# Lumina-Group/libzkp

Hardware: AMD Instinct MI355X
Metric: proofs/sec (whole node) + ms/proof p50, 4096-proof mixed batch (range / equality / membership / improvement) per MI355X (higher is better)
Workload: dtype u32/u64 integer limbs (10x25.5-bit GF(2^255-19), BN254 Fq on 9x29-bit limbs in the MSM loops and 10x26-bit elsewhere, 8x32-bit Fr and scalars mod l, 2x64-bit f128)

## Files before the change

### libzkp_amd/csrc/bn254_g.h

```cpp
#pragma once
#include "bn254_fq.h"
#include "bn254_fq9.h"

namespace zkp {

struct fq2 { fq c0, c1; };

ZKP_HD inline fq f_add(const fq& a, const fq& b) { return fq_add(a, b); }
ZKP_HD inline fq f_sub(const fq& a, const fq& b) { return fq_sub(a, b); }
ZKP_HD inline fq f_mul(const fq& a, const fq& b) { return fq_mul(a, b); }
ZKP_HD inline fq f_sq(const fq& a) { return fq_sq(a); }
ZKP_HD inline fq f_neg(const fq& a) { return fq_neg(a); }
ZKP_HD inline fq f_dbl(const fq& a) { return fq_dbl(a); }
ZKP_HD inline bool f_is_zero(const fq& a) { return fq_is_zero(a); }
ZKP_HD inline fq f_select(bool c, const fq& a, const fq& b) { return fq_select(c, a, b); }
ZKP_HD inline void f_set_zero(fq& a) { a = fq_zero(); }
ZKP_HD inline void f_set_one(fq& a) { a = fq_one(); }
ZKP_HD inline fq f_inv(const fq& a) { return fq_inv(a); }

ZKP_HD inline fq2 f_add(const fq2& a, const fq2& b) { return fq2{fq_add(a.c0, b.c0), fq_add(a.c1, b.c1)}; }
ZKP_HD inline fq2 f_sub(const fq2& a, const fq2& b) { return fq2{fq_sub(a.c0, b.c0), fq_sub(a.c1, b.c1)}; }
ZKP_HD inline fq2 f_neg(const fq2& a) { return fq2{fq_neg(a.c0), fq_neg(a.c1)}; }
ZKP_HD inline fq2 f_dbl(const fq2& a) { return fq2{fq_dbl(a.c0), fq_dbl(a.c1)}; }
ZKP_HD inline fq2 f_mul(const fq2& a, const fq2& b) {
// ... 224 lines not shown
    return h;
}
ZKP_HD inline void fr_glv_split(const uint32_t k[8], glv_half& h1, glv_half& h2) {
    const uint32_t G1[3] = {0xc7e0b3d7u, 0xd91d232eu, 0x00000002u}, G2[5] = {0x391eb18du, 0x7a7bd9d4u, 0xa773d2cfu, 0x4ccef014u, 0x00000002u};
    const uint32_t A1[2] = {0x94d213e3u, 0x89d32568u}, A2[4] = {0x1221250bu, 0x0be4e154u, 0xeeb859fdu, 0x6f4d8248u};
    const uint32_t NB1[4] = {0x7d4f1128u, 0x8211bbebu, 0xeeb859fcu, 0x6f4d8248u}, B2[2] = {0x94d213e3u, 0x89d32568u};
    uint32_t t1[11], t2[13];
    mp_mul_lo<8, 3, 11>(t1, k, G1); mp_mul_lo<8, 5, 13>(t2, k, G2);
    const uint32_t* c1 = t1 + 8;
    const uint32_t* c2 = t2 + 8;
    uint32_t p11[5], p22[5], p12[5], p21[5];
    mp_mul_lo<3, 2, 5>(p11, c1, A1); mp_mul_lo<5, 4, 5>(p22, c2, A2); mp_mul_lo<3, 4, 5>(p12, c1, NB1); mp_mul_lo<5, 2, 5>(p21, c2, B2);
    uint32_t k1[5], k2[5]; int64_t b1 = 0, b2 = 0;
    ZKP_UNROLL for (int i = 0; i < 5; i++) {
        b1 += (int64_t)k[i] - (int64_t)p11[i] - (int64_t)p22[i]; k1[i] = (uint32_t)b1; b1 >>= 32;
        b2 += (int64_t)p12[i] - (int64_t)p21[i]; k2[i] = (uint32_t)b2; b2 >>= 32;
    }
    h1 = glv_from_160(k1); h2 = glv_from_160(k2);
}
ZKP_HD inline fq fq_glv_beta() {
    const uint32_t w[8] = {0x77fffffeu, 0x57634731u, 0xacdb5c4fu, 0xd4f263f1u, 0xa0d48bacu, 0x59e26bceu, 0x00000000u, 0x00000000u};
    return fq_from_raw(w);
}
template <class F> ZKP_HD inline Jac<F> jac_mul_u128_signed(const Jac<F>& p, const uint32_t mag[4], bool neg) {
    Jac<F> tbl[8];
    tbl[0] = p; tbl[1] = jac_dbl(p);
    for (int i = 2; i < 8; i++) tbl[i] = jac_add(tbl[i - 1], p);
    int dig[33]; int carry = 0;
    for (int i = 0; i < 32; i++) {
        int v = (int)((mag[i >> 3] >> ((i & 7) * 4)) & 15u) + carry;
        carry = v > 8 ? 1 : 0; if (carry) v -= 16;
        dig[i] = v;
    }
    dig[32] = carry;
    Jac<F> acc = jac_infinity<F>();
    for (int i = 32; i >= 0; i--) {
        if (i != 32) acc = jac_dbl(jac_dbl(jac_dbl(jac_dbl(acc))));
        const int d = dig[i];
        if (d > 0) acc = jac_add(acc, tbl[d - 1]);
        else if (d < 0) acc = jac_add(acc, jac_neg(tbl[-d - 1]));
    }
    return neg ? jac_neg(acc) : acc;
}

template <class F> ZKP_HD inline bool jac_to_aff(Aff<F>& out, const Jac<F>& p) {
    if (jac_is_inf(p)) return false;
    const F zi = f_inv(p.Z), zi2 = f_sq(zi);
    out.x = f_mul(p.X, zi2); out.y = f_mul(f_mul(p.Y, zi2), zi);
    return true;
}

ZKP_HD inline bool fq_raw_gt_half(const uint32_t w[8]) {
    const uint32_t half[8] = {0x6c3e7ea3u, 0x9e10460bu, 0xb438e546u, 0xcbc0b548u, 0x40c0ac2eu, 0xdc2822dbu, 0x7098d014u, 0x18322739u};
    for (int i = 7; i >= 0; i--) { if (w[i] > half[i]) return true; if (w[i] < half[i]) return false; }
    return false;
}
ZKP_HD inline void g1_serialize(uint32_t out[16], const g1_jac& p) {
    g1_aff a;
    if (!jac_to_aff(a, p)) { for (int i = 0; i < 16; i++) out[i] = 0; out[15] = 0x40000000u; return; }
    fq_to_raw(out, a.x); fq_to_raw(out + 8, a.y);
    if (fq_raw_gt_half(out + 8)) out[15] |= 0x80000000u;
}
ZKP_HD inline void g2_serialize(uint32_t out[32], const g2_jac& p) {
    g2_aff a;
    if (!jac_to_aff(a, p)) { for (int i = 0; i < 32; i++) out[i] = 0; out[31] = 0x40000000u; return; }
// ... 8 lines not shown
```

### libzkp_amd/csrc/g16_impl.inc

```

namespace {

struct G16Key {
    bool loaded = false;
    uint32_t n_inst = 0, n_wit = 0, nv = 0, n_rows = 0, m = 0, logm = 0;
    G16Circuit C{};
    std::vector<void*> allocs;
    uint32_t *table_g1 = nullptr, *table_g2 = nullptr;
    G16Radix rx = g16_radix(G16_WBITS_DEFAULT);
    int shared_tables = -1;
    uint64_t table_bytes = 0;
    struct Chunking { DevLayout lay; const uint32_t* corr = nullptr; const uint16_t* scal = nullptr; };
    std::vector<SlotList> targets_g1, targets_g2;
    std::vector<uint16_t> hscal_g1, hscal_g2;
    std::map<uint64_t, Chunking> lays_g1, lays_g2;
    uint64_t win_g1 = 0, win_g2 = 0;
    const uint32_t *init_g1 = nullptr, *init_g2 = nullptr;
    G16Vk vk{}; bool vk_ready = false;
    uint64_t vk_table_bytes = 0;
    bool verifier_only() const { return vk_ready && !loaded; }
    const uint32_t *vm_kconst = nullptr, *vm_lines = nullptr;
};
struct G16Run {
    void* buf = nullptr; size_t cap = 0; hipStream_t side = nullptr, side2 = nullptr; hipEvent_t ev[4] = {nullptr, nullptr, nullptr, nullptr};
// ... 453 lines not shown
    hipEvent_t e1 = nullptr;
    int rc = prof_begin(K, st, &e1);
    if (rc) return rc;
    ZKP_TRACED(g2 ? "k_msm_gather<G2Msm>" : "k_msm_gather<G1Msm>", st, g16_launch_msm(g2, m, st));
    prof_end(K, st, e1, D.adds_per_row * rows);
    return 0;
}


int run_g16(int kind, uint32_t rows, const uint64_t* d_value, const uint64_t* d_set_vals, const uint32_t* d_set_len, const uint8_t* d_seeds,
            uint8_t* d_out, uint64_t stride, hipStream_t st, uint32_t lane = 0) {
    G16Key& K = g16s().key[kind];
    if (!K.loaded) return no_proving_key(K);
    const uint32_t nsc = g16_nscalars(K.nv, K.m);
    const G16Key::Chunking *c1 = nullptr, *c1c = nullptr, *c2 = nullptr;
    int rc;
    if ((rc = get_chunking(K, false, G16_PART_AB, rows, &c1)) || (rc = get_chunking(K, true, G16_PART_ALL, rows, &c2))) return rc;
    if ((rc = get_chunking(K, false, G16_PART_C, rows, &c1c))) return rc;
    size_t off = 0;
    auto sz = [&](size_t bytes) { size_t o = off; off += align_up(bytes); return o; };
    const size_t W = (size_t)32 * rows;
    const size_t o_z = sz(W * K.nv), o_sd = sz((size_t)K.rx.digw * 4 * rows * nsc), o_rs = sz(W * 2), o_p1 = sz((size_t)c1->lay.nchunks * G1_JAC_W * 4 * rows),
                 o_p1c = sz((size_t)c1c->lay.nchunks * G1_JAC_W * 4 * rows), o_p2 = sz((size_t)c2->lay.nchunks * G2_JAC_W * 4 * rows),
                 o_s1 = sz((size_t)3 * G1_JAC_W * 4 * rows), o_s2 = sz((size_t)G2_JAC_W * 4 * rows), o_t1 = sz((size_t)G16_CPARTS * G1_JAC_W * 4 * rows),
                 o_qe = sz((size_t)2 * 9 * K.m * 4 * rows);
    G16Run& RW = g16s().run[kind][lane & 1u];
    if (off > RW.cap) {
        if (RW.buf) { HIP_TRY(hipDeviceSynchronize()); HIP_TRY(hipFree(RW.buf)); RW.buf = nullptr; RW.cap = 0; }
        HIP_TRY(hipMalloc(&RW.buf, off)); RW.cap = off;
    }
    uint8_t* base = (uint8_t*)RW.buf;
    G16View V{}; V.rx = K.rx; V.rows = rows; V.kind = (uint32_t)kind; V.n_inst = K.n_inst; V.n_wit = K.n_wit; V.nv = K.nv; V.m = K.m;
    V.value = d_value; V.set_vals = d_set_vals; V.set_len = d_set_len; V.seeds = reinterpret_cast<const uint32_t*>(d_seeds); V.mimc_c = g16s().mimc_dev;
    V.z = (uint32_t*)(base + o_z); V.sdig = (uint32_t*)(base + o_sd); V.rs = (uint32_t*)(base + o_rs); V.out = d_out; V.stride = stride;
    V.qap_evals = (uint32_t*)(base + o_qe);
    uint32_t *p1 = (uint32_t*)(base + o_p1), *p1c = (uint32_t*)(base + o_p1c), *p2 = (uint32_t*)(base + o_p2), *s1 = (uint32_t*)(base + o_s1), *s2 = (uint32_t*)(base + o_s2), *t1 = (uint32_t*)(base + o_t1);
    if (!RW.last) {
        for (auto& e : RW.ev) HIP_TRY(hipEventCreateWithFlags(&e, hipEventDisableTiming));
        HIP_TRY(hipEventCreateWithFlags(&RW.last, hipEventDisableTiming));
    }
    G16Run& R0 = g16s().run[kind][0];
    if (!R0.side) {
        static const int side_level = env_int("ZKP_HIP_G16_SIDE_PRIORITY", 2), side2_level = env_int("ZKP_HIP_G16_SIDE2_PRIORITY", 0);
        HIP_TRY(hipStreamCreateWithPriority(&R0.side, hipStreamNonBlocking, stream_priority(side_level)));
        HIP_TRY(hipStreamCreateWithPriority(&R0.side2, hipStreamNonBlocking, stream_priority(side2_level)));
    }
    hipStream_t const side = R0.side, side2 = R0.side2;
    hipEvent_t ev_wit = RW.ev[0], ev_ab = RW.ev[1], ev_c = RW.ev[2], ev_cp = RW.ev[3];
    ReduceView R2{}; R2.rows = rows; R2.ntargets = 1; R2.partial = p2; R2.target_chunk_begin = c2->lay.target_chunk_begin; R2.corr = c2->corr;
    if (RW.used) HIP_TRY(hipStreamWaitEvent(st, RW.last, 0));
    ZKP_TRACED("k_g16_witness", st, g16_launch_witness(V, st));
    ZKP_TRACED("k_g16_zdigits", st, g16_launch_zdigits(V, st));
    HIP_TRY(hipEventRecord(ev_wit, st));
    HIP_TRY(hipStreamWaitEvent(side, ev_wit, 0));
    { TraceMark tm_("k_g16_qap", side); HIP_TRY(g16_launch_qap(V, K.C, side)); }
    if ((rc = launch_msm_key(false, K.rx, *c1c, K.table_g1, K.init_g1, rows, V.sdig, p1c, side))) return rc;
    ReduceView Rc{}; Rc.rows = rows; Rc.ntargets = 1; Rc.partial = p1c; Rc.target_chunk_begin = c1c->lay.target_chunk_begin; Rc.corr = c1c->corr;
    ZKP_TRACED("k_sum_t<G1Msm>", side, g16_launch_sum(false, Rc, s1 + (size_t)2 * G1_JAC_W * rows, side));
    HIP_TRY(hipEventRecord(ev_c, side));
    if ((rc = launch_msm_key(false, K.rx, *c1, K.table_g1, K.init_g1, rows, V.sdig, p1, st))) return rc;
    ReduceView Rab{}; Rab.rows = rows; Rab.ntargets = 2; Rab.partial = p1; Rab.target_chunk_begin = c1->lay.target_chunk_begin; Rab.corr = c1->corr;
    HIP_TRY(hipEventRecord(ev_ab, st));
    HIP_TRY(hipStreamWaitEvent(side2, ev_ab, 0));
    ZKP_TRACED("k_sum_t<G1Msm>", side2, g16_launch_sum(false, Rab, s1, side2));
    ZKP_TRACED("k_g16_cparts", side2, g16_launch_cparts(V, s1, t1, side2));
    HIP_TRY(hipEventRecord(ev_cp, side2));
    if ((rc = launch_msm_key(true, K.rx, *c2, K.table_g2, K.init_g2, rows, V.sdig, p2, st))) return rc;
    ZKP_TRACED("k_sum_t<G2Msm>", st, g16_launch_sum(true, R2, s2, st));
    HIP_TRY(hipStreamWaitEvent(st, ev_c, 0));
    HIP_TRY(hipStreamWaitEvent(st, ev_cp, 0));
    ZKP_TRACED("k_g16_final", st, g16_launch_final(V, s1, s2, t1, st));
    HIP_TRY(hipGetLastError());
    HIP_TRY(hipEventRecord(RW.last, st)); RW.used = true;
    return 0;
}
// ... 243 lines not shown
```

### libzkp_amd/csrc/g16_kernels.hip

```cpp
#include "g16_launch.h"
#include "msm_kernel.h"

struct G1Msm {
    static constexpr uint32_t ACC_W = G1_JAC_W, DIG_PER_WORD = 2;
    static __device__ __forceinline__ int32_t digit(uint32_t word, uint32_t w) { return (int32_t)(int16_t)(word >> (16 * (w & 1u))); }
    using Acc = g1_jac;
    static __device__ __forceinline__ Acc identity() { return jac_infinity<fq>(); }
    static constexpr uint32_t GATHER_WAVES = 3; static constexpr int GATHER_PREFETCH = 2;
    static constexpr uint32_t GATHER_W = 16, GATHER_STRIDE = 16, GATHER_PRIO = 0;
    using GAcc = g1_xyzz9;
    static __device__ __forceinline__ GAcc to_gather(const g1_jac& a) { return xyzz9_from_jac(a); }
    static __device__ __forceinline__ g1_jac from_gather(const GAcc& a) { return jac_from_xyzz9(a); }
    static __device__ __forceinline__ GAcc accumulate_entry(const GAcc& acc, int32_t d, const uint32_t* e) {
        g1_aff9 q{fq9_unpack8(e), fq9_unpack8(e + 8)};
        q.y = fq9_select(d < 0, fq9_neg_k<4>(q.y), q.y);
        return g1_mmadd9(acc, q);
    }
    static __device__ __forceinline__ void store(uint32_t* p, uint32_t idx, uint32_t row, uint32_t rows, const Acc& a) { st_g1_jac(p, idx, row, rows, a); }
    static __device__ __forceinline__ Acc load(const uint32_t* p, uint32_t idx, uint32_t row, uint32_t rows) { return ld_g1_jac(p, idx, row, rows); }
    static __device__ __forceinline__ Acc add(const Acc& a, const Acc& b) { return jac_add(a, b); }
};
struct G2Msm {
    static constexpr uint32_t ACC_W = G2_JAC_W, DIG_PER_WORD = 2;
    static __device__ __forceinline__ int32_t digit(uint32_t word, uint32_t w) { return (int32_t)(int16_t)(word >> (16 * (w & 1u))); }
    using Acc = g2_jac;
    static __device__ __forceinline__ Acc identity() { return jac_infinity<fq2>(); }
    static constexpr uint32_t GATHER_WAVES = 2; static constexpr int GATHER_PREFETCH = -1;
    static constexpr uint32_t GATHER_W = 32, GATHER_STRIDE = 32, GATHER_PRIO = 0;
    using GAcc = g2_xyzz9;
    static __device__ __forceinline__ GAcc to_gather(const g2_jac& a) { return g2_xyzz9_from_jac(a); }
    static __device__ __forceinline__ g2_jac from_gather(const GAcc& a) { return jac_from_g2_xyzz9(a); }
    static __device__ __forceinline__ GAcc accumulate_entry(const GAcc& acc, int32_t d, const uint32_t* e) {
        const g2_aff9 q{fq2_9{fq9_unpack8(e), fq9_unpack8(e + 8)}, fq2_9{fq9_unpack8(e + 16), fq9_unpack8(e + 24)}};
        return g2_mmadd9(acc, q, d < 0);
    }
    static __device__ __forceinline__ void store(uint32_t* p, uint32_t idx, uint32_t row, uint32_t rows, const Acc& a) { st_g2_jac(p, idx, row, rows, a); }
    static __device__ __forceinline__ Acc load(const uint32_t* p, uint32_t idx, uint32_t row, uint32_t rows) { return ld_g2_jac(p, idx, row, rows); }
    static __device__ __forceinline__ Acc add(const Acc& a, const Acc& b) { return jac_add(a, b); }
};


__global__ void __launch_bounds__(TW) k_g16_witness(G16View V) {
    ZKP_RAISE_PRIO();
    const uint32_t row = blockIdx.x * TW + threadIdx.x;
    if (row < V.rows) step_g16_witness(V, row);
}
__global__ void __launch_bounds__(TB) k_g16_zdigits(G16View V) {
    ZKP_RAISE_PRIO();
    const uint32_t row = blockIdx.x * TB + threadIdx.x;
    if (row < V.rows) step_g16_zdigits(V, blockIdx.y, row);
}
struct DevSync { __device__ __forceinline__ void operator()() const { __syncthreads(); } };
static constexpr int QAP_TB_MAX = 256;
__global__ void __launch_bounds__(QAP_TB_MAX) k_g16_qap(G16View V, G16Circuit C) {
    extern __shared__ uint32_t g16_lds[];
    G16Lds L; L.base = g16_lds; L.m = C.m;
    g16_qap_proof(V, C, L, V.qap_evals + (size_t)blockIdx.x * 2 * 9 * C.m, blockIdx.x, threadIdx.x, blockDim.x, DevSync());
}
__global__ void __launch_bounds__(TW) k_g16_cparts(G16View V, const uint32_t* sum_g1, uint32_t* tmp_g1) {
    ZKP_RAISE_PRIO();
    const uint32_t row = blockIdx.x * TW + threadIdx.x;
    if (row < V.rows) step_g16_cparts(V, sum_g1, tmp_g1, blockIdx.y, row);
}
__global__ void __launch_bounds__(TW) k_g16_final(G16View V, const uint32_t* sum_g1, const uint32_t* sum_g2, const uint32_t* tmp_g1) {
    ZKP_RAISE_PRIO();
    const uint32_t row = blockIdx.x * TW + threadIdx.x;
    if (row < V.rows) step_g16_final(V, sum_g1, sum_g2, tmp_g1, blockIdx.y, row);
}
__global__ void __launch_bounds__(TW) k_mimc_commit(const uint64_t* values, uint32_t n, const uint32_t* mimc_c, uint8_t* out) {
    const uint32_t i = blockIdx.x * TW + threadIdx.x;
    if (i >= n) return;
    G16View V{}; V.mimc_c = mimc_c; V.z = nullptr;
    const fr h = g16_mimc_chain(V, 0, fp_from_u64<FrParams>(values[i]), 0);
    uint32_t w[8]; fp_to_raw(w, h);
    g16_put_bytes(out + 32ull * i, w, 8);
}
constexpr uint32_t G16_TABLE_SEG = 512;
template <class F, uint32_t AFF_W>
__global__ void __launch_bounds__(TW, 2) k_g16_build_table(const uint32_t* bases, uint32_t nslots, uint32_t* table, uint32_t fmt9, G16Radix rx) {
    const uint32_t seg_len = rx.nent < G16_TABLE_SEG ? rx.nent : G16_TABLE_SEG, nseg = rx.nent / seg_len, slot_seg = rx.slot_ent / seg_len;
    const uint32_t t = blockIdx.x * TW + threadIdx.x;
    if (t >= nslots * slot_seg) return;
    const uint32_t slot = t / slot_seg, sg = t % slot_seg;
    uint32_t win = sg / nseg, seg = sg % nseg;
    if (rx.uneven && sg >= 16u * nseg) { win = sg < 18u * nseg ? 16u : 17u; seg = sg - (win == 16u ? 16u : 18u) * nseg; }
// ... 36 lines not shown
            }
            for (uint32_t j = 0; j < FW; j++) { o[j] = ax[j]; o[FW + j] = ay[j]; }
        }
    }
}



__global__ void __launch_bounds__(TW) k_g16_serialize(bool g2, const uint32_t* jac, uint32_t rows, uint8_t* out) {
    const uint32_t row = blockIdx.x * TW + threadIdx.x;
    if (row >= rows) return;
    if (!g2) { uint32_t w[16]; g1_serialize(w, ld_g1_jac(jac, 0, row, rows)); g16_put_bytes(out + 64ull * row, w, 16); }
    else { uint32_t w[32]; g2_serialize(w, ld_g2_jac(jac, 0, row, rows)); g16_put_bytes(out + 128ull * row, w, 32); }
}

template __global__ void k_msm_gather<G1Msm>(MsmView, uint32_t, uint32_t);
template __global__ void k_msm_gather<G2Msm>(MsmView, uint32_t, uint32_t);
static constexpr uint32_t G16_SUM_ROWS = 8, G16_SUM_TB = 256;
template __global__ void k_sum_t<G1Msm, G16_SUM_ROWS, G16_SUM_TB>(ReduceView, uint32_t*);
template __global__ void k_sum_t<G2Msm, G16_SUM_ROWS, G16_SUM_TB>(ReduceView, uint32_t*);
template __global__ void k_g16_build_table<fq, 20>(const uint32_t*, uint32_t, uint32_t*, uint32_t, G16Radix);
template __global__ void k_g16_build_table<fq2, 40>(const uint32_t*, uint32_t, uint32_t*, uint32_t, G16Radix);

void g16_launch_witness(const G16View& V, hipStream_t st) { k_g16_witness<<<(V.rows + TW - 1) / TW, TW, 0, st>>>(V); }
void g16_launch_zdigits(const G16View& V, hipStream_t st) { k_g16_zdigits<<<dim3((V.rows + TB - 1) / TB, V.nv), TB, 0, st>>>(V); }
hipError_t g16_launch_qap(const G16View& V, const G16Circuit& C, hipStream_t st) {
    const size_t lds = (size_t)9 * C.m * 4;
    const uint32_t tb = C.m / 4;
    if (tb < 64 || tb > (uint32_t)QAP_TB_MAX || (tb & 63u)) return hipErrorInvalidValue;
    k_g16_qap<<<V.rows, tb, lds, st>>>(V, C);
    return hipSuccess;
}
void g16_launch_cparts(const G16View& V, const uint32_t* sum_g1, uint32_t* tmp_g1, hipStream_t st) {
    k_g16_cparts<<<dim3((V.rows + TW - 1) / TW, G16_CPARTS), TW, 0, st>>>(V, sum_g1, tmp_g1);
}
void g16_launch_final(const G16View& V, const uint32_t* sum_g1, const uint32_t* sum_g2, const uint32_t* tmp_g1, hipStream_t st) {
    k_g16_final<<<dim3((V.rows + TW - 1) / TW, 3), TW, 0, st>>>(V, sum_g1, sum_g2, tmp_g1);
}
void g16_launch_mimc(const uint64_t* values, uint32_t n, const uint32_t* mimc_c, uint8_t* out, hipStream_t st) { k_mimc_commit<<<(n + TW - 1) / TW, TW, 0, st>>>(values, n, mimc_c, out); }
void g16_launch_build_table(bool g2, const uint32_t* bases, uint32_t nslots, uint32_t* table, hipStream_t st, bool msm_form, const G16Radix& rx) {
    const uint32_t seg_len = rx.nent < G16_TABLE_SEG ? rx.nent : G16_TABLE_SEG;
    const uint32_t threads = nslots * (rx.slot_ent / seg_len);
    if (!g2) k_g16_build_table<fq, 20><<<(threads + TW - 1) / TW, TW, 0, st>>>(bases, nslots, table, msm_form ? 1u : 0u, rx);
    else k_g16_build_table<fq2, 40><<<(threads + TW - 1) / TW, TW, 0, st>>>(bases, nslots, table, msm_form ? 1u : 0u, rx);
}
uint32_t g16_table_entry_words(bool g2, bool msm_form) { return msm_form ? (g2 ? G2Msm::GATHER_W : G1Msm::GATHER_W) : (g2 ? 40u : 20u); }
uint32_t g16_msm_rows_per_block(bool) { return 256u; }
uint32_t g16_msm_blocks_per_cu(bool g2) { return g2 ? G2Msm::GATHER_WAVES : G1Msm::GATHER_WAVES; }
void g16_launch_msm(bool g2, const MsmView& m, hipStream_t st) {
    const uint32_t ngroups = (m.rows + 255u) / 256u, nblocks = m.nchunks * ngroups, grid = ((nblocks + 7) / 8) * 8;
    if constexpr (gather_lds_bytes<G2Msm>() > 0 || gather_lds_bytes<G1Msm>() > 0) {
        if (gather_lds_bytes<G1Msm>()) (void)hipFuncSetAttribute(reinterpret_cast<const void*>(k_msm_gather<G1Msm>), hipFuncAttributeMaxDynamicSharedMemorySize, (int)gather_lds_bytes<G1Msm>());
        if (gather_lds_bytes<G2Msm>()) (void)hipFuncSetAttribute(reinterpret_cast<const void*>(k_msm_gather<G2Msm>), hipFuncAttributeMaxDynamicSharedMemorySize, (int)gather_lds_bytes<G2Msm>());
    }
    if (!g2) k_msm_gather<G1Msm><<<grid, 256, gather_lds_bytes<G1Msm>(), st>>>(m, ngroups, nblocks);
    else k_msm_gather<G2Msm><<<grid, 256, gather_lds_bytes<G2Msm>(), st>>>(m, ngroups, nblocks);
}
// ... 7 lines not shown
```

### libzkp_amd/csrc/g16_launch.h

```cpp
#pragma once
#include <hip/hip_runtime.h>
#include "g16_steps.h"
#include "bp_steps.h"

void g16_launch_witness(const zkp::G16View& V, hipStream_t st);
void g16_launch_zdigits(const zkp::G16View& V, hipStream_t st);
hipError_t g16_launch_qap(const zkp::G16View& V, const zkp::G16Circuit& C, hipStream_t st);
void g16_launch_cparts(const zkp::G16View& V, const uint32_t* sum_g1, uint32_t* tmp_g1, hipStream_t st);
void g16_launch_final(const zkp::G16View& V, const uint32_t* sum_g1, const uint32_t* sum_g2, const uint32_t* tmp_g1, hipStream_t st);
void g16_launch_mimc(const uint64_t* values, uint32_t n, const uint32_t* mimc_c, uint8_t* out, hipStream_t st);
void g16_launch_build_table(bool g2, const uint32_t* bases, uint32_t nslots, uint32_t* table, hipStream_t st, bool msm_form, const zkp::G16Radix& rx);
uint32_t g16_table_entry_words(bool g2, bool msm_form);
uint32_t g16_msm_rows_per_block(bool g2);
uint32_t g16_msm_blocks_per_cu(bool g2);
void g16_launch_msm(bool g2, const zkp::MsmView& m, hipStream_t st);
void g16_launch_sum(bool g2, const zkp::ReduceView& R, uint32_t* sums, hipStream_t st);
void g16_launch_serialize(bool g2, const uint32_t* jac, uint32_t rows, uint8_t* out, hipStream_t st);
```

### libzkp_amd/csrc/g16_steps.h

```cpp
#pragma once
#include "bn254_g.h"
#include "bn254_fr9.h"
#include "keccak.h"
#include "sc25519.h"

namespace zkp {

struct G16Radix { uint32_t wbits, nwin, nent, digw, nwin_u64, uneven, slot_ent; };
constexpr uint32_t G16_UNEVEN_TOP_ENT = 25088;
ZKP_HD inline G16Radix g16_radix(uint32_t wbits, bool uneven = false) {
    G16Radix r; r.wbits = wbits; r.nwin = (254 + wbits) / wbits; r.nent = 1u << (wbits - 1); r.nwin_u64 = (64 + wbits) / wbits; r.uneven = 0;
    r.slot_ent = r.nwin * r.nent;
    if (uneven && wbits == 14) { r.uneven = 1; r.nwin = 18; r.slot_ent = 18u * r.nent + G16_UNEVEN_TOP_ENT; }
    r.digw = (r.nwin + 1) / 2;
    return r;
}
ZKP_HD inline uint32_t g16_win_bit(const G16Radix& rx, uint32_t w) { return rx.uneven && w == 17 ? 239u : rx.wbits * w; }
ZKP_HD inline uint32_t g16_win_off(const G16Radix& rx, uint32_t w) { return (w + (rx.uneven && w == 17 ? 1u : 0u)) * rx.nent; }
ZKP_HD inline uint32_t g16_win_ent(const G16Radix& rx, uint32_t w) { return !rx.uneven || w < 16 ? rx.nent : w == 16 ? 2u * rx.nent : G16_UNEVEN_TOP_ENT; }
constexpr uint32_t G16_WBITS_DEFAULT = 14, G16_WBITS_KNEE = 13, G16_WBITS_MIN = 8, G16_WBITS_MAX = 15, G16_DIGW_MAX = 16;
static_assert(G16_WBITS_DEFAULT >= G16_WBITS_MIN && G16_WBITS_DEFAULT <= G16_WBITS_MAX, "key-table radix out of range");
ZKP_HD inline void g16_recode_uneven(uint32_t* packed, const sc& raw) {
    uint32_t carry = 0;
    ZKP_UNROLL for (int j = 0; j < 18; j++) {
// ... 57 lines not shown
    uint32_t* z;
    uint32_t* sdig;
    uint32_t* rs;
    uint32_t* qap_evals;
    uint8_t* out; uint64_t stride;
};
ZKP_HD inline uint32_t g16_sc_h(const G16View& V) { return V.nv; }
ZKP_HD inline uint32_t g16_sc_r(const G16View& V) { return V.nv + V.m - 1; }
ZKP_HD inline uint32_t g16_sc_s(const G16View& V) { return V.nv + V.m; }
ZKP_HD inline uint32_t g16_sc_nrs(const G16View& V) { return V.nv + V.m + 1; }
ZKP_HD inline uint32_t g16_sc_one(const G16View& V) { return V.nv + V.m + 2; }
ZKP_HD inline uint32_t g16_nscalars(uint32_t nv, uint32_t m) { return nv + m + 3; }

ZKP_HD inline fr g16_mimc_chain(const G16View& V, uint32_t row, fr x, uint32_t wit0) {
    for (uint32_t i = 0; i < MIMC_ROUNDS; i++) {
        const fr t = fp_add(x, ld_fr_c(V.mimc_c, i));
        const fr t2 = fp_sq(t), t4 = fp_sq(t2);
        x = fp_mul(t4, t);
        if (V.z) { st_fr(V.z, wit0 + 3 * i, row, V.rows, t2); st_fr(V.z, wit0 + 3 * i + 1, row, V.rows, t4); st_fr(V.z, wit0 + 3 * i + 2, row, V.rows, x); }
    }
    return x;
}

ZKP_HD inline void step_g16_witness(const G16View& V, uint32_t row) {
    const uint32_t rows = V.rows;
    const uint64_t val = V.value[row];
    const fr one = fp_one<FrParams>(), zero = fp_zero<FrParams>();
    const fr v = fp_from_u64<FrParams>(val);
    uint8_t* o = V.out + (uint64_t)row * V.stride;
    st_fr(V.z, 0, row, rows, one);
    fr h;
    uint32_t proof_len = 256;
    if (V.kind == G16_EQUALITY) {
        st_fr(V.z, 2, row, rows, v); st_fr(V.z, 3, row, rows, v);
        h = g16_mimc_chain(V, row, v, 4);
        st_fr(V.z, 1, row, rows, h);
        o[0] = 2; o[1] = 2;
    } else {
        const uint32_t len = V.set_len[row];
        const uint64_t* sv = V.set_vals + (size_t)row * G16_MAX_SET;
        const uint32_t w0 = V.n_inst;
        st_fr(V.z, w0, row, rows, v);
        h = g16_mimc_chain(V, row, v, w0 + 1);
        st_fr(V.z, 1, row, rows, h);
        uint32_t pos = 0xffffffffu;
        for (uint32_t i = 0; i < len; i++) if (pos == 0xffffffffu && sv[i] == val) pos = i;
        const uint32_t sel0 = w0 + 1 + 3 * MIMC_ROUNDS;
        for (uint32_t i = 0; i < G16_MAX_SET; i++) {
            const bool real = i < len;
            const fr si = fp_from_u64<FrParams>(real ? sv[i] : 0);
            st_fr(V.z, 2 + i, row, rows, si);
            st_fr(V.z, 2 + G16_MAX_SET + i, row, rows, real ? one : zero);
            const bool sel = i == pos;
            st_fr(V.z, sel0 + i, row, rows, sel ? one : zero);
            st_fr(V.z, sel0 + G16_MAX_SET + i, row, rows, (sel && !real) ? one : zero);
            st_fr(V.z, sel0 + 2 * G16_MAX_SET + i, row, rows, sel ? fp_sub(v, si) : zero);
        }
        o[0] = 2; o[1] = 4;
        proof_len = 4 + 8 * len + 256;
        uint8_t* pl = o + 10;
        pl[0] = (uint8_t)len; pl[1] = (uint8_t)(len >> 8); pl[2] = (uint8_t)(len >> 16); pl[3] = (uint8_t)(len >> 24);
        for (uint32_t i = 0; i < len; i++) for (int k = 0; k < 8; k++) pl[4 + 8 * i + k] = (uint8_t)(sv[i] >> (8 * k));
    }
    for (int k = 0; k < 4; k++) { o[2 + k] = (uint8_t)(proof_len >> (8 * k)); o[6 + k] = (uint8_t)(32u >> (8 * k)); }
    uint32_t hraw[8]; fp_to_raw(hraw, h);
    g16_put_bytes(o + 10 + proof_len, hraw, 8);
    uint32_t seed[8]; ZKP_UNROLL for (int k = 0; k < 8; k++) seed[k] = V.seeds[(size_t)row * 8 + k];
    uint32_t w[16];
    tape_draw64(w, seed, G16_TAPE_IDX, 0); const fr r = fp_from_wide<FrParams>(w);
    tape_draw64(w, seed, G16_TAPE_IDX, 1); const fr s = fp_from_wide<FrParams>(w);
    st_fr_digits(V.sdig, g16_sc_r(V), row, rows, r, V.rx);
    st_fr_digits(V.sdig, g16_sc_s(V), row, rows, s, V.rx);
    st_fr_digits(V.sdig, g16_sc_nrs(V), row, rows, fp_neg(fp_mul(r, s)), V.rx);
    uint32_t* q = V.sdig + (size_t)g16_sc_one(V) * V.rx.digw * rows + row;
    q[0] = 1u; for (uint32_t k = 1; k < V.rx.digw; k++) q[(size_t)k * rows] = 0u;
    fr rr, sr; fp_to_raw(rr.v, r); fp_to_raw(sr.v, s);
    st_fr(V.rs, 0, row, rows, rr); st_fr(V.rs, 1, row, rows, sr);
}
ZKP_HD inline void step_g16_zdigits(const G16View& V, uint32_t k, uint32_t row) {
    st_fr_digits(V.sdig, k, row, V.rows, ld_fr(V.z, k, row, V.rows), V.rx);
}

struct G16Circuit {
    uint32_t n_rows, m, logm;
    const uint32_t *a_ptr, *a_col, *a_coef, *b_ptr, *b_col, *b_coef, *c_ptr, *c_col, *c_coef;
    const uint32_t *tw, *tw_inv;
    const uint32_t *coset, *coset_inv;
    const uint32_t* zinv;
};
ZKP_HD inline fr g16_row_dot(const uint32_t* ptr, const uint32_t* col, const uint32_t* coef, uint32_t r, const uint32_t* z, uint32_t row, uint32_t rows) {
    fr acc = fp_zero<FrParams>();
    for (uint32_t e = ptr[r]; e < ptr[r + 1]; e++) acc = fp_add(acc, fp_mul(ld_fr_c(coef, e), ld_fr(z, col[e], row, rows)));
    return acc;
}
ZKP_HD inline uint32_t g16_bitrev(uint32_t x, uint32_t bits) {
    uint32_t r = 0; for (uint32_t i = 0; i < bits; i++) { r = (r << 1) | (x & 1u); x >>= 1; } return r;
}

struct G16Lds {
    uint32_t* base; uint32_t m;
// ... 99 lines not shown
ZKP_HD inline void st_fq_col(uint32_t* q, uint32_t rows, const fq& a) { ZKP_UNROLL for (int k = 0; k < 10; k++) q[(size_t)k * rows] = a.v[k]; }
ZKP_HD inline g1_jac ld_g1_jac(const uint32_t* p, uint32_t idx, uint32_t row, uint32_t rows) {
    const uint32_t* q = p + (size_t)idx * G1_JAC_W * rows + row; const size_t s = (size_t)10 * rows;
    g1_jac r; r.X = ld_fq_col(q, rows); r.Y = ld_fq_col(q + s, rows); r.Z = ld_fq_col(q + 2 * s, rows);
    return r;
}
ZKP_HD inline void st_g1_jac(uint32_t* p, uint32_t idx, uint32_t row, uint32_t rows, const g1_jac& g) {
    uint32_t* q = p + (size_t)idx * G1_JAC_W * rows + row; const size_t s = (size_t)10 * rows;
    st_fq_col(q, rows, g.X); st_fq_col(q + s, rows, g.Y); st_fq_col(q + 2 * s, rows, g.Z);
}
ZKP_HD inline g2_jac ld_g2_jac(const uint32_t* p, uint32_t idx, uint32_t row, uint32_t rows) {
    const uint32_t* q = p + (size_t)idx * G2_JAC_W * rows + row; const size_t s = (size_t)10 * rows;
    g2_jac r;
    r.X.c0 = ld_fq_col(q, rows); r.X.c1 = ld_fq_col(q + s, rows); r.Y.c0 = ld_fq_col(q + 2 * s, rows); r.Y.c1 = ld_fq_col(q + 3 * s, rows);
    r.Z.c0 = ld_fq_col(q + 4 * s, rows); r.Z.c1 = ld_fq_col(q + 5 * s, rows);
    return r;
}
ZKP_HD inline void st_g2_jac(uint32_t* p, uint32_t idx, uint32_t row, uint32_t rows, const g2_jac& g) {
    uint32_t* q = p + (size_t)idx * G2_JAC_W * rows + row; const size_t s = (size_t)10 * rows;
    st_fq_col(q, rows, g.X.c0); st_fq_col(q + s, rows, g.X.c1); st_fq_col(q + 2 * s, rows, g.Y.c0); st_fq_col(q + 3 * s, rows, g.Y.c1);
    st_fq_col(q + 4 * s, rows, g.Z.c0); st_fq_col(q + 5 * s, rows, g.Z.c1);
}
constexpr uint32_t G16_CPARTS = 4;
ZKP_HD inline void step_g16_cparts(const G16View& V, const uint32_t* sum_g1, uint32_t* tmp_g1, uint32_t part, uint32_t row) {
    const uint32_t rows = V.rows, which = part >> 1;
    g1_jac P = ld_g1_jac(sum_g1, which, row, rows);
    const fr k = ld_fr(V.rs, which == 0 ? 1 : 0, row, rows);
    glv_half h1, h2; fr_glv_split(k.v, h1, h2);
    if (part & 1u) P.X = fq_mul(P.X, fq_glv_beta());
    const glv_half& h = (part & 1u) ? h2 : h1;
    st_g1_jac(tmp_g1, part, row, rows, jac_mul_u128_signed(P, h.mag, h.neg));
}
ZKP_HD inline void step_g16_final(const G16View& V, const uint32_t* sum_g1, const uint32_t* sum_g2, const uint32_t* tmp_g1, uint32_t which, uint32_t row) {
    const uint32_t rows = V.rows;
    uint8_t* o = V.out + (uint64_t)row * V.stride;
    uint32_t plen = 0; for (int k = 0; k < 4; k++) plen |= (uint32_t)o[2 + k] << (8 * k);
    uint8_t* pr = o + 10 + plen - 256;
    if (which == 0) {
        uint32_t w1[16]; g1_serialize(w1, ld_g1_jac(sum_g1, 0, row, rows)); g16_put_bytes(pr, w1, 16);
    } else if (which == 1) {
        uint32_t w2[32]; g2_serialize(w2, ld_g2_jac(sum_g2, 0, row, rows)); g16_put_bytes(pr + 64, w2, 32);
    } else {
        g1_jac Cc = ld_g1_jac(sum_g1, 2, row, rows);
        for (uint32_t t = 0; t < G16_CPARTS; t++) Cc = jac_add(Cc, ld_g1_jac(tmp_g1, t, row, rows));
        uint32_t w1[16]; g1_serialize(w1, Cc); g16_put_bytes(pr + 192, w1, 16);
    }
}

}
```

Measured before the change: 336,700.

## Parallelize Groth16 witness MiMC chain across threads and move C-part tables to LDS

The witness kernel now runs each row's MiMC chain in a block with helper threads that spill the intermediate round values (t^2, t^4, x) to global memory and also write their scalar digits, so the separate zdigits kernel is gone. Per-set auxiliary witness entries are split into independent per-element tasks. For the C-part scalar muls, the 8-entry Jacobian precompute table now sits in shared memory in column layout instead of registers/scratch, the signed 4-bit recoding is computed on the fly, and the four partial products are summed inside the block, so only one temp point is written per row. The intent is to cut register pressure and scratch spills, one launch, and global traffic for the temp points. The cost is larger shared-memory use per block, which may limit occupancy, plus extra barrier synchronisation.

```diff
diff --git a/libzkp_amd/csrc/bn254_g.h b/libzkp_amd/csrc/bn254_g.h
--- a/libzkp_amd/csrc/bn254_g.h
+++ b/libzkp_amd/csrc/bn254_g.h
@@ -270,25 +270,49 @@
     const uint32_t w[8] = {0x77fffffeu, 0x57634731u, 0xacdb5c4fu, 0xd4f263f1u, 0xa0d48bacu, 0x59e26bceu, 0x00000000u, 0x00000000u};
     return fq_from_raw(w);
 }
+struct G1TblCol {
+    uint32_t* base; uint32_t nl;
+    ZKP_HD void st(uint32_t i, const Jac<fq>& p) const {
+        uint32_t* q = base + (size_t)30 * i * nl;
+        ZKP_UNROLL for (int k = 0; k < 10; k++) { q[(size_t)k * nl] = p.X.v[k]; q[(size_t)(10 + k) * nl] = p.Y.v[k]; q[(size_t)(20 + k) * nl] = p.Z.v[k]; }
+    }
+    ZKP_HD Jac<fq> ld(uint32_t i) const {
+        const uint32_t* q = base + (size_t)30 * i * nl; Jac<fq> p;
+        ZKP_UNROLL for (int k = 0; k < 10; k++) { p.X.v[k] = q[(size_t)k * nl]; p.Y.v[k] = q[(size_t)(10 + k) * nl]; p.Z.v[k] = q[(size_t)(20 + k) * nl]; }
+        return p;
+    }
+};
+constexpr uint32_t G1_TBL_WORDS = 8 * 30;
+ZKP_HD inline Jac<fq> jac_mul_u128_tbl(const Jac<fq>& p, const uint32_t mag[4], bool neg, const G1TblCol& tbl) {
+    {
+        Jac<fq> t = jac_dbl(p);
+        tbl.st(0, p); tbl.st(1, t);
+        for (uint32_t i = 2; i < 8; i++) { t = jac_add(t, p); tbl.st(i, t); }
+    }
+    uint32_t w0, w1, w2, w3, top;
+    {
+        uint64_t c = (uint64_t)mag[0] + 0x88888888u; w0 = (uint32_t)c;
+        c = (c >> 32) + mag[1] + 0x88888888u; w1 = (uint32_t)c;
+        c = (c >> 32) + mag[2] + 0x88888888u; w2 = (uint32_t)c;
+        c = (c >> 32) + mag[3] + 0x88888888u; w3 = (uint32_t)c;
+        top = (uint32_t)(c >> 32);
+    }
+    Jac<fq> acc = top ? p : jac_infinity<fq>();
+    for (int i = 0; i < 32; i++) {
+        acc = jac_dbl(jac_dbl(jac_dbl(jac_dbl(acc))));
+        const int d = (int)(w3 >> 28) - 8;
+        w3 = (w3 << 4) | (w2 >> 28); w2 = (w2 << 4) | (w1 >> 28); w1 = (w1 << 4) | (w0 >> 28); w0 <<= 4;
+        if (d != 0) {
+            Jac<fq> q = tbl.ld((uint32_t)(d < 0 ? -d : d) - 1u);
+            q.Y = fq_select(d < 0, fq_neg(q.Y), q.Y);
+            acc = jac_add(acc, q);
+        }
+    }
+    return neg ? jac_neg(acc) : acc;
+}
 template <class F> ZKP_HD inline Jac<F> jac_mul_u128_signed(const Jac<F>& p, const uint32_t mag[4], bool neg) {
-    Jac<F> tbl[8];
-    tbl[0] = p; tbl[1] = jac_dbl(p);
-    for (int i = 2; i < 8; i++) tbl[i] = jac_add(tbl[i - 1], p);
-    int dig[33]; int carry = 0;
-    for (int i = 0; i < 32; i++) {
-        int v = (int)((mag[i >> 3] >> ((i & 7) * 4)) & 15u) + carry;
-        carry = v > 8 ? 1 : 0; if (carry) v -= 16;
-        dig[i] = v;
-    }
-    dig[32] = carry;
-    Jac<F> acc = jac_infinity<F>();
-    for (int i = 32; i >= 0; i--) {
-        if (i != 32) acc = jac_dbl(jac_dbl(jac_dbl(jac_dbl(acc))));
-        const int d = dig[i];
-        if (d > 0) acc = jac_add(acc, tbl[d - 1]);
-        else if (d < 0) acc = jac_add(acc, jac_neg(tbl[-d - 1]));
-    }
-    return neg ? jac_neg(acc) : acc;
+    uint32_t col[G1_TBL_WORDS];
+    return jac_mul_u128_tbl(p, mag, neg, G1TblCol{col, 1u});
 }
 
 template <class F> ZKP_HD inline bool jac_to_aff(Aff<F>& out, const Jac<F>& p) {
diff --git a/libzkp_amd/csrc/g16_impl.inc b/libzkp_amd/csrc/g16_impl.inc
--- a/libzkp_amd/csrc/g16_impl.inc
+++ b/libzkp_amd/csrc/g16_impl.inc
@@ -499,7 +499,7 @@
     const size_t W = (size_t)32 * rows;
     const size_t o_z = sz(W * K.nv), o_sd = sz((size_t)K.rx.digw * 4 * rows * nsc), o_rs = sz(W * 2), o_p1 = sz((size_t)c1->lay.nchunks * G1_JAC_W * 4 * rows),
                  o_p1c = sz((size_t)c1c->lay.nchunks * G1_JAC_W * 4 * rows), o_p2 = sz((size_t)c2->lay.nchunks * G2_JAC_W * 4 * rows),
-                 o_s1 = sz((size_t)3 * G1_JAC_W * 4 * rows), o_s2 = sz((size_t)G2_JAC_W * 4 * rows), o_t1 = sz((size_t)G16_CPARTS * G1_JAC_W * 4 * rows),
+                 o_s1 = sz((size_t)3 * G1_JAC_W * 4 * rows), o_s2 = sz((size_t)G2_JAC_W * 4 * rows), o_t1 = sz((size_t)G1_JAC_W * 4 * rows),
                  o_qe = sz((size_t)2 * 9 * K.m * 4 * rows);
     G16Run& RW = g16s().run[kind][lane & 1u];
     if (off > RW.cap) {
@@ -527,7 +527,6 @@
     ReduceView R2{}; R2.rows = rows; R2.ntargets = 1; R2.partial = p2; R2.target_chunk_begin = c2->lay.target_chunk_begin; R2.corr = c2->corr;
     if (RW.used) HIP_TRY(hipStreamWaitEvent(st, RW.last, 0));
     ZKP_TRACED("k_g16_witness", st, g16_launch_witness(V, st));
-    ZKP_TRACED("k_g16_zdigits", st, g16_launch_zdigits(V, st));
     HIP_TRY(hipEventRecord(ev_wit, st));
     HIP_TRY(hipStreamWaitEvent(side, ev_wit, 0));
     { TraceMark tm_("k_g16_qap", side); HIP_TRY(g16_launch_qap(V, K.C, side)); }
diff --git a/libzkp_amd/csrc/g16_kernels.hip b/libzkp_amd/csrc/g16_kernels.hip
--- a/libzkp_amd/csrc/g16_kernels.hip
+++ b/libzkp_amd/csrc/g16_kernels.hip
@@ -40,17 +40,14 @@
 };
 
 
-__global__ void __launch_bounds__(TW) k_g16_witness(G16View V) {
+struct DevSync { __device__ __forceinline__ void operator()() const { __syncthreads(); } };
+__global__ void __launch_bounds__(TB) k_g16_witness(G16View V, uint32_t nchain) {
+    __shared__ uint32_t lds[g16_chain_lds_words(G16_CHAIN_ROWS)];
     ZKP_RAISE_PRIO();
-    const uint32_t row = blockIdx.x * TW + threadIdx.x;
-    if (row < V.rows) step_g16_witness(V, row);
+    if (blockIdx.x < nchain) { step_g16_chain(V, lds, blockIdx.x * G16_CHAIN_ROWS, G16_CHAIN_ROWS, threadIdx.x, TB, DevSync()); return; }
+    const uint32_t a = (blockIdx.x - nchain) * TB + threadIdx.x;
+    if (a < g16_aux_tasks(V) * V.rows) step_g16_aux(V, a / V.rows, a % V.rows);
 }
-__global__ void __launch_bounds__(TB) k_g16_zdigits(G16View V) {
-    ZKP_RAISE_PRIO();
-    const uint32_t row = blockIdx.x * TB + threadIdx.x;
-    if (row < V.rows) step_g16_zdigits(V, blockIdx.y, row);
-}
-struct DevSync { __device__ __forceinline__ void operator()() const { __syncthreads(); } };
 static constexpr int QAP_TB_MAX = 256;
 __global__ void __launch_bounds__(QAP_TB_MAX) k_g16_qap(G16View V, G16Circuit C) {
     extern __shared__ uint32_t g16_lds[];
@@ -59,8 +56,8 @@
 }
 __global__ void __launch_bounds__(TW) k_g16_cparts(G16View V, const uint32_t* sum_g1, uint32_t* tmp_g1) {
     ZKP_RAISE_PRIO();
-    const uint32_t row = blockIdx.x * TW + threadIdx.x;
-    if (row < V.rows) step_g16_cparts(V, sum_g1, tmp_g1, blockIdx.y, row);
+    __shared__ uint32_t tbl[G1_TBL_WORDS * TW];
+    step_g16_cparts(V, sum_g1, tmp_g1, tbl, blockIdx.x * (TW / G16_CPARTS), TW, threadIdx.x, TW, DevSync());
 }
 __global__ void __launch_bounds__(TW) k_g16_final(G16View V, const uint32_t* sum_g1, const uint32_t* sum_g2, const uint32_t* tmp_g1) {
     ZKP_RAISE_PRIO();
@@ -143,8 +140,10 @@
 template __global__ void k_g16_build_table<fq, 20>(const uint32_t*, uint32_t, uint32_t*, uint32_t, G16Radix);
 template __global__ void k_g16_build_table<fq2, 40>(const uint32_t*, uint32_t, uint32_t*, uint32_t, G16Radix);
 
-void g16_launch_witness(const G16View& V, hipStream_t st) { k_g16_witness<<<(V.rows + TW - 1) / TW, TW, 0, st>>>(V); }
-void g16_launch_zdigits(const G16View& V, hipStream_t st) { k_g16_zdigits<<<dim3((V.rows + TB - 1) / TB, V.nv), TB, 0, st>>>(V); }
+void g16_launch_witness(const G16View& V, hipStream_t st) {
+    const uint32_t nchain = (V.rows + G16_CHAIN_ROWS - 1) / G16_CHAIN_ROWS, naux = (g16_aux_tasks(V) * V.rows + TB - 1) / TB;
+    k_g16_witness<<<nchain + naux, TB, 0, st>>>(V, nchain);
+}
 hipError_t g16_launch_qap(const G16View& V, const G16Circuit& C, hipStream_t st) {
     const size_t lds = (size_t)9 * C.m * 4;
     const uint32_t tb = C.m / 4;
@@ -153,7 +152,8 @@
     return hipSuccess;
 }
 void g16_launch_cparts(const G16View& V, const uint32_t* sum_g1, uint32_t* tmp_g1, hipStream_t st) {
-    k_g16_cparts<<<dim3((V.rows + TW - 1) / TW, G16_CPARTS), TW, 0, st>>>(V, sum_g1, tmp_g1);
+    constexpr uint32_t rows_per = TW / G16_CPARTS;
+    k_g16_cparts<<<(V.rows + rows_per - 1) / rows_per, TW, 0, st>>>(V, sum_g1, tmp_g1);
 }
 void g16_launch_final(const G16View& V, const uint32_t* sum_g1, const uint32_t* sum_g2, const uint32_t* tmp_g1, hipStream_t st) {
     k_g16_final<<<dim3((V.rows + TW - 1) / TW, 3), TW, 0, st>>>(V, sum_g1, sum_g2, tmp_g1);
diff --git a/libzkp_amd/csrc/g16_launch.h b/libzkp_amd/csrc/g16_launch.h
--- a/libzkp_amd/csrc/g16_launch.h
+++ b/libzkp_amd/csrc/g16_launch.h
@@ -4,7 +4,6 @@
 #include "bp_steps.h"
 
 void g16_launch_witness(const zkp::G16View& V, hipStream_t st);
-void g16_launch_zdigits(const zkp::G16View& V, hipStream_t st);
 hipError_t g16_launch_qap(const zkp::G16View& V, const zkp::G16Circuit& C, hipStream_t st);
 void g16_launch_cparts(const zkp::G16View& V, const uint32_t* sum_g1, uint32_t* tmp_g1, hipStream_t st);
 void g16_launch_final(const zkp::G16View& V, const uint32_t* sum_g1, const uint32_t* sum_g2, const uint32_t* tmp_g1, hipStream_t st);
diff --git a/libzkp_amd/csrc/g16_steps.h b/libzkp_amd/csrc/g16_steps.h
--- a/libzkp_amd/csrc/g16_steps.h
+++ b/libzkp_amd/csrc/g16_steps.h
@@ -103,49 +103,77 @@
     return x;
 }
 
-ZKP_HD inline void step_g16_witness(const G16View& V, uint32_t row) {
+ZKP_HD inline void st_z(const G16View& V, uint32_t k, uint32_t row, const fr& x) { st_fr(V.z, k, row, V.rows, x); st_fr_digits(V.sdig, k, row, V.rows, x, V.rx); }
+ZKP_HD inline void st_z_bit(const G16View& V, uint32_t k, uint32_t row, bool bit) {
+    st_fr(V.z, k, row, V.rows, bit ? fp_one<FrParams>() : fp_zero<FrParams>());
+    uint32_t* q = V.sdig + (size_t)k * V.rx.digw * V.rows + row;
+    q[0] = bit ? 1u : 0u; for (uint32_t j = 1; j < V.rx.digw; j++) q[(size_t)j * V.rows] = 0u;
+}
+ZKP_HD inline uint32_t g16_wit0(const G16View& V) { return V.kind == G16_EQUALITY ? 4u : V.n_inst + 1u; }
+ZKP_HD inline uint32_t g16_proof_len(const G16View& V, uint32_t row) { return V.kind == G16_EQUALITY ? 256u : 4u + 8u * V.set_len[row] + 256u; }
+ZKP_HD inline uint32_t g16_aux_tasks(const G16View& V) { return V.kind == G16_EQUALITY ? 1u : 1u + G16_MAX_SET; }
+constexpr uint32_t G16_CHAIN_ROWS = 64;
+ZKP_HD constexpr uint32_t g16_chain_lds_words(uint32_t rb) { return 2u * 3u * 8u * rb; }
+template <class Sync>
+ZKP_HD inline void step_g16_chain(const G16View& V, uint32_t* lds, uint32_t row0, uint32_t rb, uint32_t tid, uint32_t nthreads, Sync sync) {
+    const bool chains = tid < rb, helps = nthreads == rb || tid >= rb;
+    const uint32_t hid = nthreads == rb ? tid : tid - rb, nh = nthreads == rb ? nthreads : nthreads - rb;
+    const uint32_t row = row0 + tid, wit0 = g16_wit0(V);
+    const bool live = chains && row < V.rows;
+    fr x = live ? fp_from_u64<FrParams>(V.value[row]) : fp_zero<FrParams>();
+    for (uint32_t i = 0; i < MIMC_ROUNDS; i++) {
+        uint32_t* buf = lds + (size_t)(i & 1u) * 24 * rb;
+        if (chains) {
+            const fr t = fp_add(x, ld_fr_c(V.mimc_c, i));
+            const fr t2 = fp_sq(t), t4 = fp_sq(t2);
+            x = fp_mul(t4, t);
+            ZKP_UNROLL for (int k = 0; k < 8; k++) { buf[(size_t)k * rb + tid] = t2.v[k]; buf[(size_t)(8 + k) * rb + tid] = t4.v[k]; buf[(size_t)(16 + k) * rb + tid] = x.v[k]; }
+        }
+        sync();
+        if (helps) for (uint32_t t = hid; t < 3 * rb; t += nh) {
+            const uint32_t var = t / rb, r = t % rb;
+            if (row0 + r >= V.rows) continue;
+            fr y; ZKP_UNROLL for (int k = 0; k < 8; k++) y.v[k] = buf[(size_t)(8 * var + k) * rb + r];
+            st_z(V, wit0 + 3 * i + var, row0 + r, y);
+        }
+    }
+    if (!live) return;
+    st_z(V, 1, row, x);
+    uint32_t hraw[8]; fp_to_raw(hraw, x);
+    g16_put_bytes(V.out + (uint64_t)row * V.stride + 10 + g16_proof_len(V, row), hraw, 8);
+}
+ZKP_HD inline void step_g16_aux(const G16View& V, uint32_t task, uint32_t row) {
     const uint32_t rows = V.rows;
     const uint64_t val = V.value[row];
-    const fr one = fp_one<FrParams>(), zero = fp_zero<FrParams>();
     const fr v = fp_from_u64<FrParams>(val);
     uint8_t* o = V.out + (uint64_t)row * V.stride;
-    st_fr(V.z, 0, row, rows, one);
-    fr h;
-    uint32_t proof_len = 256;
+    if (task != 0) {
+        const uint32_t i = task - 1, len = V.set_len[row], sel0 = V.n_inst + 1 + 3 * MIMC_ROUNDS;
+        const uint64_t* sv = V.set_vals + (size_t)row * G16_MAX_SET;
+        const bool real = i < len;
+        bool sel = real && sv[i] == val;
+        for (uint32_t j = 0; j < i && sel; j++) if (sv[j] == val) sel = false;
+        const fr si = fp_from_u64<FrParams>(real ? sv[i] : 0);
+        st_z(V, 2 + i, row, si);
+        st_z_bit(V, 2 + G16_MAX_SET + i, row, real);
+        st_z_bit(V, sel0 + i, row, sel);
+        st_z_bit(V, sel0 + G16_MAX_SET + i, row, sel && !real);
+        st_z(V, sel0 + 2 * G16_MAX_SET + i, row, sel ? fp_sub(v, si) : fp_zero<FrParams>());
+        if (real) for (int k = 0; k < 8; k++) o[14 + 8 * i + k] = (uint8_t)(sv[i] >> (8 * k));
+        return;
+    }
+    st_z_bit(V, 0, row, true);
+    const uint32_t proof_len = g16_proof_len(V, row);
     if (V.kind == G16_EQUALITY) {
-        st_fr(V.z, 2, row, rows, v); st_fr(V.z, 3, row, rows, v);
-        h = g16_mimc_chain(V, row, v, 4);
-        st_fr(V.z, 1, row, rows, h);
+        st_z(V, 2, row, v); st_z(V, 3, row, v);
         o[0] = 2; o[1] = 2;
     } else {
+        st_z(V, V.n_inst, row, v);
         const uint32_t len = V.set_len[row];
-        const uint64_t* sv = V.set_vals + (size_t)row * G16_MAX_SET;
-        const uint32_t w0 = V.n_inst;
-        st_fr(V.z, w0, row, rows, v);
-        h = g16_mimc_chain(V, row, v, w0 + 1);
-        st_fr(V.z, 1, row, rows, h);
-        uint32_t pos = 0xffffffffu;
-        for (uint32_t i = 0; i < len; i++) if (pos == 0xffffffffu && sv[i] == val) pos = i;
-        const uint32_t sel0 = w0 + 1 + 3 * MIMC_ROUNDS;
-        for (uint32_t i = 0; i < G16_MAX_SET; i++) {
-            const bool real = i < len;
-            const fr si = fp_from_u64<FrParams>(real ? sv[i] : 0);
-            st_fr(V.z, 2 + i, row, rows, si);
-            st_fr(V.z, 2 + G16_MAX_SET + i, row, rows, real ? one : zero);
-            const bool sel = i == pos;
-            st_fr(V.z, sel0 + i, row, rows, sel ? one : zero);
-            st_fr(V.z, sel0 + G16_MAX_SET + i, row, rows, (sel && !real) ? one : zero);
-            st_fr(V.z, sel0 + 2 * G16_MAX_SET + i, row, rows, sel ? fp_sub(v, si) : zero);
-        }
         o[0] = 2; o[1] = 4;
-        proof_len = 4 + 8 * len + 256;
-        uint8_t* pl = o + 10;
-        pl[0] = (uint8_t)len; pl[1] = (uint8_t)(len >> 8); pl[2] = (uint8_t)(len >> 16); pl[3] = (uint8_t)(len >> 24);
-        for (uint32_t i = 0; i < len; i++) for (int k = 0; k < 8; k++) pl[4 + 8 * i + k] = (uint8_t)(sv[i] >> (8 * k));
+        for (int k = 0; k < 4; k++) o[10 + k] = (uint8_t)(len >> (8 * k));
     }
     for (int k = 0; k < 4; k++) { o[2 + k] = (uint8_t)(proof_len >> (8 * k)); o[6 + k] = (uint8_t)(32u >> (8 * k)); }
-    uint32_t hraw[8]; fp_to_raw(hraw, h);
-    g16_put_bytes(o + 10 + proof_len, hraw, 8);
     uint32_t seed[8]; ZKP_UNROLL for (int k = 0; k < 8; k++) seed[k] = V.seeds[(size_t)row * 8 + k];
     uint32_t w[16];
     tape_draw64(w, seed, G16_TAPE_IDX, 0); const fr r = fp_from_wide<FrParams>(w);
@@ -157,6 +185,12 @@
     q[0] = 1u; for (uint32_t k = 1; k < V.rx.digw; k++) q[(size_t)k * rows] = 0u;
     fr rr, sr; fp_to_raw(rr.v, r); fp_to_raw(sr.v, s);
     st_fr(V.rs, 0, row, rows, rr); st_fr(V.rs, 1, row, rows, sr);
+}
+struct G16NoSync { ZKP_HD void operator()() const {} };
+ZKP_HD inline void step_g16_witness(const G16View& V, uint32_t row) {
+    uint32_t lds[g16_chain_lds_words(1)];
+    step_g16_chain(V, lds, row, 1, 0, 1, G16NoSync());
+    for (uint32_t task = 0; task < g16_aux_tasks(V); task++) step_g16_aux(V, task, row);
 }
 ZKP_HD inline void step_g16_zdigits(const G16View& V, uint32_t k, uint32_t row) {
     st_fr_digits(V.sdig, k, row, V.rows, ld_fr(V.z, k, row, V.rows), V.rx);
@@ -302,14 +336,33 @@
     st_fq_col(q + 4 * s, rows, g.Z.c0); st_fq_col(q + 5 * s, rows, g.Z.c1);
 }
 constexpr uint32_t G16_CPARTS = 4;
-ZKP_HD inline void step_g16_cparts(const G16View& V, const uint32_t* sum_g1, uint32_t* tmp_g1, uint32_t part, uint32_t row) {
+ZKP_HD inline void g16_cpart_mul(const G16View& V, const uint32_t* sum_g1, const G1TblCol& col, uint32_t part, uint32_t row) {
     const uint32_t rows = V.rows, which = part >> 1;
     g1_jac P = ld_g1_jac(sum_g1, which, row, rows);
     const fr k = ld_fr(V.rs, which == 0 ? 1 : 0, row, rows);
     glv_half h1, h2; fr_glv_split(k.v, h1, h2);
     if (part & 1u) P.X = fq_mul(P.X, fq_glv_beta());
-    const glv_half& h = (part & 1u) ? h2 : h1;
-    st_g1_jac(tmp_g1, part, row, rows, jac_mul_u128_signed(P, h.mag, h.neg));
+    const bool second = (part & 1u) != 0;
+    const uint32_t mag[4] = {second ? h2.mag[0] : h1.mag[0], second ? h2.mag[1] : h1.mag[1], second ? h2.mag[2] : h1.mag[2], second ? h2.mag[3] : h1.mag[3]};
+    col.st(0, jac_mul_u128_tbl(P, mag, second ? h2.neg : h1.neg, col));
+}
+ZKP_HD inline g1_jac g16_cpart_join(const G1TblCol& col, uint32_t off) { return jac_add(col.ld(0), G1TblCol{col.base + off, col.nl}.ld(0)); }
+template <class Sync>
+ZKP_HD inline void step_g16_cparts(const G16View& V, const uint32_t* sum_g1, uint32_t* tmp_g1, uint32_t* tbl, uint32_t row0, uint32_t nlanes, uint32_t tid, uint32_t nthreads, Sync sync) {
+    for (uint32_t l = tid; l < nlanes; l += nthreads) {
+        const uint32_t row = row0 + l / G16_CPARTS;
+        if (row < V.rows) g16_cpart_mul(V, sum_g1, G1TblCol{tbl + l, nlanes}, l % G16_CPARTS, row);
+    }
+    sync();
+    for (uint32_t l = tid; l < nlanes; l += nthreads) {
+        const G1TblCol col{tbl + l, nlanes};
+        if (row0 + l / G16_CPARTS < V.rows && (l & 1u) == 0) col.st(0, g16_cpart_join(col, 1));
+    }
+    sync();
+    for (uint32_t l = tid; l < nlanes; l += nthreads) {
+        const uint32_t row = row0 + l / G16_CPARTS;
+        if (row < V.rows && l % G16_CPARTS == 0) st_g1_jac(tmp_g1, 0, row, V.rows, g16_cpart_join(G1TblCol{tbl + l, nlanes}, 2));
+    }
 }
 ZKP_HD inline void step_g16_final(const G16View& V, const uint32_t* sum_g1, const uint32_t* sum_g2, const uint32_t* tmp_g1, uint32_t which, uint32_t row) {
     const uint32_t rows = V.rows;
@@ -321,10 +374,8 @@
     } else if (which == 1) {
         uint32_t w2[32]; g2_serialize(w2, ld_g2_jac(sum_g2, 0, row, rows)); g16_put_bytes(pr + 64, w2, 32);
     } else {
-        g1_jac Cc = ld_g1_jac(sum_g1, 2, row, rows);
-        for (uint32_t t = 0; t < G16_CPARTS; t++) Cc = jac_add(Cc, ld_g1_jac(tmp_g1, t, row, rows));
-        uint32_t w1[16]; g1_serialize(w1, Cc); g16_put_bytes(pr + 192, w1, 16);
-    }
-}
-
-}
+        uint32_t w1[16]; g1_serialize(w1, jac_add(ld_g1_jac(sum_g1, 2, row, rows), ld_g1_jac(tmp_g1, 0, row, rows))); g16_put_bytes(pr + 192, w1, 16);
+    }
+}
+
+}
```

Result: no change. 338,900 (median of 5 runs) (+0.7%).
